# jcorsetti/oryon

Hardware: AMD Instinct MI355X
Metric: image-pairs/sec end-to-end (feat+match+reg) @224², C=256; ADD(-S) parity (higher is better)
Workload: dtype f32

## Files before the change

### include/oryon_hip.h

```cpp
#ifndef ORYON_HIP_H
#define ORYON_HIP_H

#include <stddef.h>
#include <stdint.h>

#ifdef __cplusplus
extern "C" {
#endif

#define ORYON_OK 0
#define ORYON_ERR_INVALID_ARG (-1)
#define ORYON_ERR_HIP (-2)
#define ORYON_ERR_WORKSPACE (-3)
#define ORYON_ERR_NO_DEVICE (-4)
#define ORYON_ERR_STATE (-5)

#define ORYON_PAIR_OK 0
#define ORYON_PAIR_NO_MASK 1
#define ORYON_PAIR_NO_CORR 2

#define ORYON_MATCH_TILE 128

const char *oryon_version(void);
const char *oryon_last_error(void);
// ... 248 lines not shown
    int n_slots;
    int overlap;
    int gather_sets;
    int reg_streams;
    int reg_lag;
    int screen;
    int sample_first;
    int x3_prefetch;
    int stream_roles;
    int screen_cascade;
    int solver;
    int ransac_max_iter;
    float ransac_match_err;
    float ransac_fix_percent;
} oryon_engine_config_t;
size_t oryon_engine_config_bytes(void);
size_t oryon_engine_arena_bytes(const oryon_engine_config_t *cfg, const oryon_pointdsc_t *solver);
int oryon_engine_create(oryon_engine_t **handle, const oryon_engine_config_t *cfg, oryon_pointdsc_t *solver, void *arena,
                        size_t arena_bytes);
void oryon_engine_destroy(oryon_engine_t *handle);
int oryon_engine_warm_streams(void);
int oryon_engine_set_stream_roles(oryon_engine_t *handle, int roles);
int oryon_engine_stream_roles(const oryon_engine_t *handle, int *roles);
int oryon_engine_buffer(const oryon_engine_t *handle, int slot, const char *name, size_t *offset, size_t *bytes);
int oryon_engine_geometry(const oryon_engine_t *handle, int *cap_a, int *cap_q, int *c_pad, int *n_cap);
int oryon_engine_submit(oryon_engine_t *handle, const float *feat_a, const float *feat_q, const int32_t *mask_a, const int32_t *mask_q,
                        const float *depth_a, const float *depth_q, const float *cam_a, const float *cam_q, const int64_t *pair_key,
                        int force_eager, int inputs_resident, void *caller_stream);
int oryon_engine_wait(oryon_engine_t *handle, int slot, void *caller_stream);
int oryon_engine_set_timing(oryon_engine_t *handle, int enable);
int oryon_engine_timing(oryon_engine_t *handle, int64_t step, float *out8);
int oryon_engine_elapsed(oryon_engine_t *handle, int64_t step_a, int event_a, int64_t step_b, int event_b, float *ms);
int oryon_engine_gather_ms(oryon_engine_t *handle, int64_t step, float *ms);
int oryon_engine_host_stats(const oryon_engine_t *handle, int64_t *n_submit, double *submit_ms_total, double *submit_ms_last);
int oryon_engine_x3_steps(const oryon_engine_t *handle, int64_t *n_steps);
int oryon_engine_cascade_stats(oryon_engine_t *handle, int32_t *out);
int oryon_engine_feedback(oryon_engine_t *handle, int64_t *step, int64_t *n_undecided, int64_t *n_anchors);

int oryon_split_f16x3(const float *x, int64_t n, void *hi_f16, void *lo_f16, void *stream);
int oryon_x3_range_flag(int *value_out, int reset, void *stream);
int oryon_linear_f16x3(const float *A, int M, int K, const void *W_hi, const void *W_lo, const float *bias, int N, int act, float *C,
                       void *stream);
int oryon_linear_f16x3_acc(const float *A, int M, int K, const void *W_hi, const void *W_lo, const float *bias, int N, float *C,
                           void *stream);

int oryon_mha_f16x3(const float *qkv, int N, int L, int heads, int head_dim, float *out, void *stream);
// ... 98 lines not shown
```

### oryon_amd/_lib.py

```python
from __future__ import annotations

import ctypes
import os
from ctypes import POINTER, c_char_p, c_float, c_int, c_int64, c_size_t, c_uint64, c_void_p

import torch

_HERE = os.path.dirname(os.path.abspath(__file__))
LIB_PATH = os.path.join(_HERE, "liboryon_hip.so")
_lib = None


class OryonError(RuntimeError):
    pass


class EngineConfig(ctypes.Structure):
    _fields_ = [("B", c_int), ("C", c_int), ("FH", c_int), ("FW", c_int), ("HA", c_int), ("WA", c_int), ("HQ", c_int), ("WQ", c_int),
                ("layout", c_int), ("dist_th", c_float), ("n_corrs", c_int), ("src_sampling", c_int), ("seed", c_uint64),
                ("round_f16", c_int), ("n_slots", c_int), ("overlap", c_int), ("gather_sets", c_int), ("reg_streams", c_int), ("reg_lag", c_int), ("screen", c_int), ("sample_first", c_int), ("x3_prefetch", c_int), ("stream_roles", c_int), ("screen_cascade", c_int),
                ("solver", c_int), ("ransac_max_iter", c_int), ("ransac_match_err", c_float), ("ransac_fix_percent", c_float)]


class DecoderWeights(ctypes.Structure):
# ... 86 lines not shown
                                   _P, _P, _P, _P, _P]),
    "oryon_lift_pairs": (c_int, [_P, _P, c_int, c_int, c_int, c_int, _P, c_int, c_int, _P, c_int, c_int, _P, _P, _P, _P,
                                 _P, _P, _P]),
    "oryon_lift_points": (c_int, [_P, c_int, c_int, _P, _P, _P, c_int, _P, _P]),
    "oryon_kabsch_batched": (c_int, [_P, _P, _P, c_int, c_int, _P, _P]),
    "oryon_split_f16x3": (c_int, [_P, c_int64, _P, _P, _P]),
    "oryon_linear_f16x3": (c_int, [_P, c_int, c_int, _P, _P, _P, c_int, c_int, _P, _P]),
    "oryon_linear_f16x3_acc": (c_int, [_P, c_int, c_int, _P, _P, _P, c_int, _P, _P]),
    "oryon_mha_f16x3": (c_int, [_P, c_int, c_int, c_int, c_int, _P, _P]),
    "oryon_pose_metrics": (c_int, [_P, _P, c_int, _P, _P, c_int, c_int, _P, _P, _P, _P]),
    "oryon_pose_bop_workspace_bytes": (c_size_t, [c_int, c_int]),
    "oryon_pose_bop_errors": (c_int, [_P, _P, _P, c_int, _P, _P, _P, _P, c_int, c_int, _P, c_int, _P, _P, _P]),
    "oryon_render_depth_workspace_bytes": (c_size_t, [c_int, c_int]),
    "oryon_render_depth": (c_int, [_P, _P, c_int, _P, _P, _P, _P, c_int, c_int, _P, c_int, c_int, _P, _P, _P]),
    "oryon_vsd_workspace_bytes": (c_size_t, [c_int, c_int, c_int, c_int]),
    "oryon_vsd_counts": (c_int, [_P, _P, _P, _P, c_int, c_int, c_int, _P, _P, _P, _P, c_int, c_int, _P, _P, ctypes.c_double, _P, c_int,
                                 _P, _P, _P]),
    "oryon_engine_arena_bytes": (c_size_t, [POINTER(EngineConfig), c_void_p]),
    "oryon_engine_create": (c_int, [POINTER(c_void_p), POINTER(EngineConfig), c_void_p, _P, c_size_t]),
    "oryon_engine_destroy": (None, [c_void_p]),
    "oryon_engine_warm_streams": (c_int, []),
    "oryon_engine_set_stream_roles": (c_int, [c_void_p, c_int]),
    "oryon_engine_stream_roles": (c_int, [c_void_p, POINTER(c_int)]),
    "oryon_engine_buffer": (c_int, [c_void_p, c_int, c_char_p, POINTER(c_size_t), POINTER(c_size_t)]),
    "oryon_engine_geometry": (c_int, [c_void_p, POINTER(c_int), POINTER(c_int), POINTER(c_int), POINTER(c_int)]),
    "oryon_engine_submit": (c_int, [c_void_p, _P, _P, _P, _P, _P, _P, _P, _P, _P, c_int, c_int, _P]),
    "oryon_engine_wait": (c_int, [c_void_p, c_int, _P]),
    "oryon_engine_set_timing": (c_int, [c_void_p, c_int]),
    "oryon_engine_timing": (c_int, [c_void_p, c_int64, POINTER(c_float)]),
    "oryon_engine_elapsed": (c_int, [c_void_p, c_int64, c_int, c_int64, c_int, POINTER(c_float)]),
    "oryon_engine_gather_ms": (c_int, [c_void_p, c_int64, POINTER(c_float)]),
    "oryon_engine_config_bytes": (c_size_t, []),
    "oryon_engine_host_stats": (c_int, [c_void_p, POINTER(c_int64), POINTER(ctypes.c_double), POINTER(ctypes.c_double)]),
    "oryon_engine_x3_steps": (c_int, [c_void_p, POINTER(c_int64)]),
    "oryon_engine_cascade_stats": (c_int, [c_void_p, c_void_p]),
    "oryon_engine_feedback": (c_int, [_P, POINTER(c_int64), POINTER(c_int64), POINTER(c_int64)]),
    "oryon_fusion_window_attention_f32": (c_int, [_P, _P, c_int, c_int, c_int, c_int, c_int, c_int, c_int, _P, _P]),
    "oryon_fusion_class_layer_f32": (c_int, [_P, _P, POINTER(FusionClassWeights), c_int, _P, _P]),
    "oryon_conv24_image_bytes": (c_int64, [c_int, c_int, c_int]),
    "oryon_conv24_pack_f16x3": (c_int, [_P, c_int, c_int, c_int, _P, _P]),
    "oryon_conv24_f16x3": (c_int, [_P, c_int, c_int, _P, _P, c_int, c_int, c_int, _P, _P]),
    "oryon_decoder_create": (c_int, [POINTER(DecoderWeights), POINTER(c_void_p), _P]),
    "oryon_decoder_destroy": (None, [c_void_p]),
    "oryon_decoder_workspace_bytes": (c_int64, [c_int, c_int, c_int]),
    "oryon_decoder_workspace_layout": (c_int, [c_int, c_int, c_int, POINTER(c_int64)]),
    "oryon_decoder_forward": (c_int, [c_void_p, _P, _P, _P, c_int, c_int, c_int, _P, c_int64, _P, _P, c_int, c_int, _P]),
# ... 100 lines not shown
```

### oryon_amd/csrc/engine.hip

```cpp
#include <stdlib.h>
#include <chrono>
#include <new>
#include <vector>
#include <string.h>
#include "common.h"
#include "match_common.h"

using namespace oryon;

namespace {
constexpr int MAX_SLOTS = 8;
constexpr int MAX_G_SLOTS = 4;
constexpr int MAX_REG_STREAMS = 4;
constexpr int TIMING_RING = 64;
constexpr int ROW_PAD = 256;
constexpr int POOL_STREAMS = 8;
constexpr int DEFAULT_ROLES = 2345;

inline bool roles_valid(int roles)
{
    if (roles < 0 || roles > 7777) return false;
    for (int d = 0, r = roles; d < 4; ++d, r /= 10)
        if (r % 10 >= POOL_STREAMS) return false;
    return true;
// ... 28 lines not shown

struct Named {
    const char *name;
    size_t off, bytes;
};

struct Layout {
    GatherBuf gbuf[MAX_G_SLOTS];
    SlotBuf slot[MAX_SLOTS];
    std::vector<Named> names[MAX_SLOTS];
    void *match_ws;
    size_t match_ws_bytes, pdsc_ws_bytes, bytes;
    int cap_a, cap_q, c_pad, n_cap, cap_a1;
};
}

struct oryon_engine {
    oryon_engine_config_t cfg;
    oryon_pointdsc_t *solver;
    char *arena;
    Layout L;
    int device;
    hipStream_t sg, sm, sr[MAX_REG_STREAMS];
    int n_reg_streams;
    int roles;
    hipEvent_t ev_inputs[MAX_SLOTS], ev_gathered[MAX_SLOTS], ev_matched[MAX_SLOTS], ev_done[MAX_SLOTS];
    hipEvent_t tev[TIMING_RING][9];
    bool timed[TIMING_RING];
    bool used[MAX_SLOTS];
    bool timing;
    int32_t *fb_host;
    hipEvent_t ev_fb[MAX_SLOTS];
    int64_t fb_step[MAX_SLOTS];
    int64_t fb_seen;
    bool hard_mode;
    int64_t n_x3;
    int64_t n_submit;
    double host_ns_total, host_ns_last;
};

namespace {
int carve_engine(const oryon_engine_config_t &c, const oryon_pointdsc_t *solver, char *base, Layout &L)
{
    const int HW = c.FH * c.FW;
    L.c_pad = c.C <= 256 ? 256 : 512;
    const int keep = c.src_sampling > 0 ? (c.src_sampling < HW ? c.src_sampling : HW) : HW;
    L.cap_a = (int)up((size_t)keep, ROW_PAD);
    L.cap_q = (int)up((size_t)HW, ROW_PAD);
    L.n_cap = (int)up((size_t)c.n_corrs, 128);
// ... 139 lines not shown
        out[i] = pool.all[i];
    }
    return hipSuccess;
}
}

extern "C" int oryon_engine_warm_streams(void)
{
    int dev = 0;
    ORYON_CHECK_HIP(hipGetDevice(&dev));
    hipStream_t tmp[POOL_STREAMS];
    ORYON_CHECK_HIP(acquire_pool(dev, tmp));
    return ORYON_OK;
}

namespace {
int assign_roles(oryon_engine *e, int roles)
{
    hipStream_t pool[POOL_STREAMS];
    ORYON_CHECK_HIP(acquire_pool(e->device, pool));
    const int r_m = roles / 1000 % 10, r_g = roles / 100 % 10, r_r0 = roles / 10 % 10, r_r1 = roles % 10;
    e->sm = e->cfg.overlap >= 1 ? pool[r_m] : nullptr;
    e->sg = e->cfg.overlap >= 2 ? pool[r_g] : nullptr;
    for (int s = 0; s < MAX_REG_STREAMS; ++s) e->sr[s] = nullptr;
    for (int s = 0; s < e->n_reg_streams; ++s)
        if (e->cfg.overlap >= 1) e->sr[s] = pool[(s == 0 ? r_r0 : s == 1 ? r_r1 : 2 + s) & 7];
    e->roles = roles;
    return ORYON_OK;
}
}

extern "C" int oryon_engine_create(oryon_engine_t **handle, const oryon_engine_config_t *cfg, oryon_pointdsc_t *solver, void *arena,
                                   size_t arena_bytes)
{
    ORYON_CHECK_ARG(handle && arena);
    int rc = check_cfg(cfg);
    if (rc) return rc;
    ORYON_CHECK_ARG(solver || cfg->solver == 1);
    oryon_engine *e = new (std::nothrow) oryon_engine();
    ORYON_CHECK_ARG(e != nullptr);
    e->cfg = *cfg;
    e->solver = solver;
    e->arena = static_cast<char *>(arena);
    if ((rc = carve_engine(*cfg, solver, e->arena, e->L))) { delete e; set_error("oryon_engine_create: cannot size the workspaces (solver finalized?)"); return rc; }
    if (arena_bytes < e->L.bytes) {
        set_error("oryon_engine_create: arena too small (%zu < %zu)", arena_bytes, e->L.bytes);
        delete e;
        return ORYON_ERR_WORKSPACE;
    }
    (void)hipGetDevice(&e->device);
    {
        hipPointerAttribute_t attr;
        if (hipPointerGetAttributes(&attr, arena) == hipSuccess && attr.device != e->device) {
            set_error("oryon_engine_create: the arena lives on device %d, the calling thread is on device %d", attr.device, e->device);
            delete e;
            return ORYON_ERR_INVALID_ARG;
        }
        (void)hipGetLastError();
    }
    e->sg = e->sm = nullptr;
    e->timing = false;
    e->n_submit = 0;
    e->fb_host = nullptr;
    e->fb_seen = -1;
    e->hard_mode = false;
    e->n_x3 = 0;
    for (int s = 0; s < MAX_SLOTS; ++s) { e->ev_fb[s] = nullptr; e->fb_step[s] = -1; }
    e->host_ns_total = e->host_ns_last = 0.0;
    hipError_t err = hipSuccess;
    auto ok = [&](hipError_t x) { if (err == hipSuccess) err = x; };
    e->n_reg_streams = cfg->reg_streams;
    for (int s = 0; s < MAX_REG_STREAMS; ++s) e->sr[s] = nullptr;
    if (assign_roles(e, cfg->stream_roles > 0 ? cfg->stream_roles : DEFAULT_ROLES) != ORYON_OK)
        err = hipErrorUnknown;
    for (int s = 0; s < MAX_SLOTS; ++s) {
        e->used[s] = false;
        e->ev_inputs[s] = e->ev_gathered[s] = e->ev_matched[s] = e->ev_done[s] = nullptr;
    }
    for (int r = 0; r < TIMING_RING; ++r) {
        e->timed[r] = false;
        for (int i = 0; i < 9; ++i) e->tev[r][i] = nullptr;
    }
    for (int s = 0; s < cfg->n_slots; ++s) {
        for (hipEvent_t *ev : {&e->ev_inputs[s], &e->ev_gathered[s], &e->ev_matched[s], &e->ev_done[s]})
            ok(hipEventCreateWithFlags(ev, hipEventDisableTiming));
    }
    for (int r = 0; r < TIMING_RING; ++r)
        for (int i = 0; i < 9; ++i) ok(hipEventCreate(&e->tev[r][i]));
    if (cfg->x3_prefetch && e->L.c_pad == 256) {
        ok(hipHostMalloc(reinterpret_cast<void **>(&e->fb_host), (size_t)MAX_SLOTS * 2 * cfg->B * sizeof(int32_t), hipHostMallocDefault));
        for (int s = 0; s < cfg->n_slots; ++s) ok(hipEventCreateWithFlags(&e->ev_fb[s], hipEventDisableTiming));
    }
    for (int s = 0; s < cfg->n_slots; ++s)
        ok(hipMemset(e->L.slot[s].corrs, 0, (size_t)cfg->B * e->L.n_cap * 4 * sizeof(int32_t)));
    ok(hipDeviceSynchronize());
    if (err != hipSuccess) {
        set_error("oryon_engine_create: stream / event creation failed: %s", hipGetErrorString(err));
        oryon_engine_destroy(e);
        return ORYON_ERR_HIP;
    }
    *handle = e;
    return ORYON_OK;
}

extern "C" void oryon_engine_destroy(oryon_engine_t *e)
{
    if (!e) return;
    for (int s = 0; s < MAX_REG_STREAMS; ++s)
        if (e->sr[s]) (void)hipStreamSynchronize(e->sr[s]);
    for (int s = 0; s < MAX_SLOTS; ++s) {
        for (hipEvent_t ev : {e->ev_inputs[s], e->ev_gathered[s], e->ev_matched[s], e->ev_done[s]})
            if (ev) (void)hipEventDestroy(ev);
    }
    for (int r = 0; r < TIMING_RING; ++r)
        for (int i = 0; i < 9; ++i)
            if (e->tev[r][i]) (void)hipEventDestroy(e->tev[r][i]);
    if (e->sm) (void)hipStreamSynchronize(e->sm);
    if (e->sg) (void)hipStreamSynchronize(e->sg);
    for (int s = 0; s < MAX_SLOTS; ++s)
        if (e->ev_fb[s]) (void)hipEventDestroy(e->ev_fb[s]);
    if (e->fb_host) (void)hipHostFree(e->fb_host);
    delete e;
}

extern "C" int oryon_engine_set_timing(oryon_engine_t *e, int enable)
{
    ORYON_CHECK_ARG(e);
    e->timing = enable != 0;
    return ORYON_OK;
}

extern "C" int oryon_engine_set_stream_roles(oryon_engine_t *e, int roles)
{
    ORYON_CHECK_ARG(e && roles_valid(roles));
    if (roles == 0) roles = DEFAULT_ROLES;
    if (e->cfg.overlap == 0 || roles == e->roles) return ORYON_OK;
    for (hipStream_t st : {e->sm, e->sg, e->sr[0], e->sr[1], e->sr[2], e->sr[3]})
        if (st) ORYON_CHECK_HIP(hipStreamSynchronize(st));
    return assign_roles(e, roles);
}

extern "C" int oryon_engine_stream_roles(const oryon_engine_t *e, int *roles)
{
    ORYON_CHECK_ARG(e && roles);
    *roles = e->roles;
    return ORYON_OK;
}

extern "C" int oryon_engine_buffer(const oryon_engine_t *e, int slot, const char *name, size_t *offset, size_t *bytes)
{
    ORYON_CHECK_ARG(e && name && offset && bytes && slot >= 0 && slot < e->cfg.n_slots);
    for (const Named &n : e->L.names[slot])
        if (strcmp(n.name, name) == 0) {
            *offset = n.off;
            *bytes = n.bytes;
            return ORYON_OK;
        }
    set_error("oryon_engine_buffer: no buffer named '%s'", name);
    return ORYON_ERR_INVALID_ARG;
}

extern "C" int oryon_engine_geometry(const oryon_engine_t *e, int *cap_a, int *cap_q, int *c_pad, int *n_cap)
{
    ORYON_CHECK_ARG(e);
    if (cap_a) *cap_a = e->L.cap_a;
    if (cap_q) *cap_q = e->L.cap_q;
    if (c_pad) *c_pad = e->L.c_pad;
    if (n_cap) *n_cap = e->L.n_cap;
    return ORYON_OK;
}

extern "C" int oryon_engine_submit(oryon_engine_t *e, const float *feat_a, const float *feat_q, const int32_t *mask_a, const int32_t *mask_q,
                                   const float *depth_a, const float *depth_q, const float *cam_a, const float *cam_q,
                                   const int64_t *pair_key, int force_eager, int inputs_resident, void *caller_stream)
{
    ORYON_CHECK_ARG(e && feat_a && feat_q && mask_a && mask_q && depth_a && depth_q && cam_a && cam_q);
    const auto t_host0 = std::chrono::steady_clock::now();
    const oryon_engine_config_t &c = e->cfg;
    const int slot = (int)(e->n_submit % c.n_slots);
    SlotBuf &b = e->L.slot[slot];
    GatherBuf &g = e->L.gbuf[e->n_submit % c.gather_sets];
    hipStream_t caller = as_stream(caller_stream);
    hipStream_t sm = c.overlap >= 1 ? e->sm : caller;
    hipStream_t sg = c.overlap >= 2 ? e->sg : sm;
    hipStream_t sr = c.overlap >= 1 ? e->sr[e->n_submit % e->n_reg_streams] : caller;
    const int HW = c.FH * c.FW, B = c.B;
    const bool timing = e->timing;
    hipEvent_t *tev = e->tev[e->n_submit % TIMING_RING];
    e->timed[e->n_submit % TIMING_RING] = timing;
    int rc;
    if (c.overlap >= 1) {
        ORYON_CHECK_HIP(hipEventRecord(e->ev_inputs[slot], caller));
        ORYON_CHECK_HIP(hipStreamWaitEvent(sr, e->ev_inputs[slot], 0));
        if (!inputs_resident || e->n_submit < c.n_slots) {
            ORYON_CHECK_HIP(hipStreamWaitEvent(sg, e->ev_inputs[slot], 0));
            if (sm != sg) ORYON_CHECK_HIP(hipStreamWaitEvent(sm, e->ev_inputs[slot], 0));
        }
        if (e->used[slot]) {
            ORYON_CHECK_HIP(hipStreamWaitEvent(sg, e->ev_done[slot], 0));
            if (sm != sg) ORYON_CHECK_HIP(hipStreamWaitEvent(sm, e->ev_done[slot], 0));
        }
        if (c.reg_lag > 0 && e->n_submit >= c.reg_lag)
            ORYON_CHECK_HIP(hipStreamWaitEvent(sm, e->ev_done[(e->n_submit - c.reg_lag) % c.n_slots], 0));
        if (sg != sm && e->n_submit >= c.gather_sets)
            ORYON_CHECK_HIP(hipStreamWaitEvent(sg, e->ev_matched[(e->n_submit - c.gather_sets) % c.n_slots], 0));
    }
    static const int ablate_env = dev_env_int("ORYON_ENGINE_ABLATE", 0);
    const int ablate = e->n_submit >= (int64_t)(c.n_slots + c.gather_sets) ? ablate_env : 0;
    if (timing) ORYON_CHECK_HIP(hipEventRecord(tev[0], sg));
    const bool mx6 = c.screen == 1 && !force_eager;
    {
        const bool clear = mx6 && !(ablate & 1);
        const bool sf_k0 = e->L.cap_a1 > 0 && !force_eager;
        if ((rc = roi_compact_pair_launch(mask_a, mask_q, B, HW, b.roi_a, b.roi_q, b.n_a, b.n_q, clear ? (sf_k0 ? g.a_eps_1 : g.a_eps) : nullptr,
                                          clear ? g.q_eps : nullptr, sg))) {
            set_error("oryon_engine_submit: roi_compact launch failed");
            return rc;
        }
    }
    if (c.src_sampling > 0 && (rc = oryon_roi_subsample(b.roi_a, b.n_a, B, HW, c.src_sampling, c.seed, pair_key, sg))) return rc;
    const bool sf = e->L.cap_a1 > 0 && !force_eager;
    const int32_t *roi_a_k0 = b.roi_a, *n_a_k0 = b.n_a;
    int cap_a_k0 = e->L.cap_a;
    int8_t *a8_k0 = g.a8;
    float *a_sc_k0 = g.a_sc, *a_eps_k0 = g.a_eps, *a_norm_k0 = g.a_norm, *a_hat_k0 = force_eager ? g.a_hat : nullptr;
    if (sf) {
        ORYON_CHECK_HIP(hipMemcpyAsync(b.roi_a1, b.roi_a, (size_t)B * HW * sizeof(int32_t), hipMemcpyDeviceToDevice, sg));
        ORYON_CHECK_HIP(hipMemcpyAsync(b.n_a1, b.n_a, (size_t)B * sizeof(int32_t), hipMemcpyDeviceToDevice, sg));
        if ((rc = oryon_roi_subsample(b.roi_a1, b.n_a1, B, HW, c.sample_first, c.seed ^ 0x5A17F125ull, pair_key, sg))) return rc;
        roi_a_k0 = b.roi_a1; n_a_k0 = b.n_a1; cap_a_k0 = e->L.cap_a1;
        a8_k0 = g.a8_1; a_sc_k0 = g.a_sc_1; a_eps_k0 = g.a_eps_1; a_norm_k0 = g.a_norm_1;
    }
    bool x3_pre = false;
    if (e->fb_host && mx6) {
        for (int s = 0; s < c.n_slots; ++s) {
            if (e->fb_step[s] > e->fb_seen && hipEventQuery(e->ev_fb[s]) == hipSuccess) {
                const int32_t *h = e->fb_host + (size_t)s * 2 * B;
                long und = 0, all = 0;
                for (int i = 0; i < B; ++i) { und += h[i]; all += h[B + i]; }
                e->hard_mode = all > 0 && 4 * und > all;
                e->fb_seen = e->fb_step[s];
            }
        }
        x3_pre = e->hard_mode && !sf && g.q_hilo != nullptr;
    }
    if (x3_pre) a_hat_k0 = g.a_hat;
    if (timing) ORYON_CHECK_HIP(hipEventRecord(tev[8], sg));
    if (ablate & 1) {
    } else if (mx6) {
        if (x3_pre) {
            if ((rc = oryon_gather_mx6_x3(feat_q, B, c.C, HW, c.layout, b.roi_q, HW, b.n_q, e->L.cap_q, e->L.c_pad, reinterpret_cast<uint8_t *>(g.q8),
                                          g.q_eps, g.q_norm, g.q_hilo, g.q_lo_max, c.round_f16, sg))) return rc;
            e->n_x3 += 1;
        } else
        if ((rc = gather_mx6_prezeroed(feat_q, B, c.C, HW, c.layout, b.roi_q, HW, b.n_q, e->L.cap_q, e->L.c_pad, reinterpret_cast<uint8_t *>(g.q8),
                                       g.q_eps, g.q_norm, nullptr, c.round_f16, sg))) return rc;
        if ((rc = gather_mx6_prezeroed(feat_a, B, c.C, HW, c.layout, roi_a_k0, HW, n_a_k0, cap_a_k0, e->L.c_pad, reinterpret_cast<uint8_t *>(a8_k0),
                                       a_eps_k0, a_norm_k0, a_hat_k0, c.round_f16, sg))) return rc;
    } else {
    if ((rc = oryon_gather_q8(feat_q, B, c.C, HW, c.layout, b.roi_q, HW, b.n_q, e->L.cap_q, e->L.c_pad, g.q8, g.q_sc, g.q_eps, g.q_norm,
                              nullptr, c.round_f16, sg))) return rc;
    if ((rc = oryon_gather_q8(feat_a, B, c.C, HW, c.layout, roi_a_k0, HW, n_a_k0, cap_a_k0, e->L.c_pad, a8_k0, a_sc_k0, a_eps_k0, a_norm_k0,
                              a_hat_k0, c.round_f16, sg))) return rc;
    }
    if (timing) ORYON_CHECK_HIP(hipEventRecord(tev[1], sg));
    if (sg != sm) {
        ORYON_CHECK_HIP(hipEventRecord(e->ev_gathered[slot], sg));
        ORYON_CHECK_HIP(hipStreamWaitEvent(sm, e->ev_gathered[slot], 0));
    }
    struct Disarm {
        bool armed = false;
        ~Disarm() { if (armed) (void)oryon_profile_events(nullptr, nullptr); }
    } disarm;
    if (timing) {
        ORYON_CHECK_HIP(hipEventRecord(tev[2], sm));
        (void)oryon_profile_events(tev[4], tev[5]);
        disarm.armed = true;
    }
    auto match_call = [&](const float *a_norm_, const int8_t *a8_, const float *a_sc_, const float *a_eps_, const int32_t *roi_a_, int cap_a_,
                          const int32_t *n_a_, int32_t *corrs_, int32_t *n_valid_, int32_t *n_sel_, int32_t *status_, int32_t *n_und_) -> int {
        MatchCorrsArgs m;
        m.a_i8 = a8_;
        m.a_scale = mx6 ? a_eps_ : a_sc_;
        m.roi_a = roi_a_;
        m.roi_stride_a = HW;
        m.feat_q = feat_q;
        m.q_norm = g.q_norm;
        m.roi_q = b.roi_q;
        m.roi_stride_q = HW;
        m.q_i8 = g.q8;
        m.q_scale = mx6 ? nullptr : g.q_sc;
        m.q_eps_max = g.q_eps;
        m.C_true = c.C;
        m.HW = HW;
        m.layout = c.layout;
        m.B = B;
        m.C = e->L.c_pad;
        m.cap_a = cap_a_;
        m.cap_q = e->L.cap_q;
        m.round_f16 = c.round_f16;
        m.n_a = n_a_;
        m.n_q = b.n_q;
        m.threshold = c.dist_th;
// ... 6 lines not shown
        m.argmin = b.argmin;
        m.valid = b.valid;
        m.corrs = corrs_;
        m.n_valid = n_valid_;
        m.n_sel = n_sel_;
        m.status = status_;
        m.n_undecided = n_und_;
        m.workspace = e->L.match_ws;
        m.workspace_bytes = e->L.match_ws_bytes;
        m.stream = sm;
        m.fmt = mx6 ? 1 : 0;
        m.cascade = (c.screen_cascade && !sf) ? 1 : 0;
        if (mx6 && x3_pre) {
            m.a_hat = g.a_hat;
            m.q_hi_lo = g.q_hilo;
            m.q_lo_sq_max = g.q_lo_max;
        } else if (force_eager) {
            m.a_hat = g.a_hat;
            m.force_eager = force_eager;
        } else {
            m.feat_a = feat_a;
            m.a_norm = a_norm_;
        }
        return match_corrs_lazy_impl(m);
    };
    if (ablate & 2) {
    } else if (sf) {
        if ((rc = match_call(g.a_norm_1, g.a8_1, g.a_sc_1, g.a_eps_1, b.roi_a1, e->L.cap_a1, b.n_a1, b.corrs, b.n_valid, b.n_sel, b.status, b.n_und)))
            return rc;
        if ((rc = oryon_sample_first_gate(b.n_valid, b.n_a1, b.n_a, B, c.n_corrs, b.n_a2, sm))) return rc;
        if (mx6) {
            if ((rc = oryon_gather_mx6(feat_a, B, c.C, HW, c.layout, b.roi_a, HW, b.n_a2, e->L.cap_a, e->L.c_pad, reinterpret_cast<uint8_t *>(g.a8),
                                       g.a_eps, g.a_norm, nullptr, c.round_f16, sm))) return rc;
        } else if ((rc = oryon_gather_q8(feat_a, B, c.C, HW, c.layout, b.roi_a, HW, b.n_a2, e->L.cap_a, e->L.c_pad, g.a8, g.a_sc, g.a_eps, g.a_norm,
                                         nullptr, c.round_f16, sm))) return rc;
        if ((rc = match_call(g.a_norm, g.a8, g.a_sc, g.a_eps, b.roi_a, e->L.cap_a, b.n_a2, b.corrs2, b.n_valid2, b.n_sel2, b.status2, nullptr)))
            return rc;
        if ((rc = oryon_sample_first_merge(b.n_a2, b.corrs2, b.n_valid2, b.n_sel2, b.status2, B, e->L.n_cap, b.corrs, b.n_valid, b.n_sel, b.status,
                                           sm))) return rc;
    } else if ((rc = match_call(g.a_norm, g.a8, g.a_sc, g.a_eps, b.roi_a, e->L.cap_a, b.n_a, b.corrs, b.n_valid, b.n_sel, b.status, b.n_und)))
        return rc;
    if (e->fb_host && mx6 && !(ablate & 2)) {
        int32_t *h = e->fb_host + (size_t)slot * 2 * B;
        ORYON_CHECK_HIP(hipMemcpyAsync(h, b.n_und, (size_t)B * sizeof(int32_t), hipMemcpyDeviceToHost, sm));
        ORYON_CHECK_HIP(hipMemcpyAsync(h + B, b.n_a, (size_t)B * sizeof(int32_t), hipMemcpyDeviceToHost, sm));
        ORYON_CHECK_HIP(hipEventRecord(e->ev_fb[slot], sm));
        e->fb_step[slot] = e->n_submit;
    }
    if (!(ablate & 2) && (rc = oryon_lift_pairs(b.corrs, b.n_sel, B, e->L.n_cap, c.FH, c.FW, depth_a, c.HA, c.WA, depth_q, c.HQ, c.WQ, cam_a, cam_q,
                                                b.status, b.pcd_a, b.pcd_q, b.n_lift, sm))) return rc;
    if (timing) ORYON_CHECK_HIP(hipEventRecord(tev[3], sm));
    if (c.overlap >= 1) {
        ORYON_CHECK_HIP(hipEventRecord(e->ev_matched[slot], sm));
        ORYON_CHECK_HIP(hipStreamWaitEvent(sr, e->ev_matched[slot], 0));
    }
    if (timing) ORYON_CHECK_HIP(hipEventRecord(tev[6], sr));
    if (c.solver == 1) {
        if (!(ablate & 4) && (rc = oryon_ransac_register(b.pcd_a, b.pcd_q, b.n_lift, B, e->L.n_cap, c.ransac_max_iter, (double)c.ransac_match_err,
                                                         (double)c.ransac_fix_percent, nullptr, c.seed, pair_key, b.status, b.pdsc_ws,
                                                         e->L.pdsc_ws_bytes, b.pose, nullptr, nullptr, nullptr, b.status_out, sr))) return rc;
    } else if (!(ablate & 4) && (rc = oryon_pointdsc_register(e->solver, b.pcd_a, b.pcd_q, b.n_lift, B, e->L.n_cap, b.status, b.pdsc_ws, e->L.pdsc_ws_bytes,
                                                       b.pose, nullptr, b.status_out, sr))) return rc;
    hipLaunchKernelGGL(engine_counts_kernel, dim3((B + 255) / 256), dim3(256), 0, sr, b.n_valid, b.n_lift, B, b.n_valid_out, b.n_lift_out);
    ORYON_CHECK_LAUNCH();
    if (timing) ORYON_CHECK_HIP(hipEventRecord(tev[7], sr));
    if (c.overlap >= 1) ORYON_CHECK_HIP(hipEventRecord(e->ev_done[slot], sr));
    e->used[slot] = true;
    e->n_submit += 1;
// ... 95 lines not shown
```

### oryon_amd/csrc/match_common.h

```cpp
#pragma once
#include <hip/hip_fp16.h>
#include "common.h"

namespace oryon {

typedef float f32x16 __attribute__((ext_vector_type(16)));

__device__ __forceinline__ void lex_min(float &d, int &i, float od, int oi)
{
    const bool take = (od < d) || (od == d && oi < i);
    d = take ? od : d;
    i = take ? oi : i;
}

int match_f32_flagged(const float *a_hat, const float *q_hat, int B, int C, int cap_a, int cap_q, const int32_t *n_a,
                      const int32_t *n_q, float threshold, float *min_dist, int32_t *argmin, uint8_t *valid,
                      const int32_t *panel_flag, const uint8_t *row_flag, void *stream);

int match_f32_split(int B, int T);

size_t match_x3_scratch_bytes(int B, int cap_s, int S, int cap_q);
size_t match_x3_zero_bytes(int B, int cap_s, int S);
int match_x3_resolve(const float *a_c, const int32_t *n_c, int cap_s, const float *feat_q, int C_true, int HW, int layout,
                     const int32_t *roi_q, int roi_stride_q, const float *q_norm, const int32_t *n_q, int B, int cap_q, float threshold,
// ... 151 lines not shown
struct MatchCorrsArgs : Screen8Args {
    const float *feat_a = nullptr;
    const float *a_norm = nullptr;
    const int32_t *roi_a = nullptr;
    int roi_stride_a = 0;
    const void *q_hi_lo = nullptr;
    const float *q_lo_sq_max = nullptr;
    const int32_t *n_a = nullptr;
    int W = 0;
    int max_corrs = 0;
    int corr_rows = 0;
    uint64_t seed = 0;
    const int64_t *pair_key = nullptr;
    int32_t *corrs = nullptr;
    int32_t *n_valid = nullptr;
    int32_t *n_sel = nullptr;
    int32_t *status = nullptr;
    int32_t *n_undecided = nullptr;
    void *workspace = nullptr;
    size_t workspace_bytes = 0;
    int fmt = 0;
    int force_eager = 0;
    int cascade = 1;
};
int match_corrs_lazy_impl(const MatchCorrsArgs &m);
int32_t *match_dc_stats(void *workspace, int B, int C, int cap_a, int cap_q, int corr_rows);

}
```

### oryon_amd/csrc/match_corrs.hip

```cpp
#include <hip/hip_fp16.h>
#include "common.h"
#include "match_common.h"
#include "match_exact.h"

namespace oryon {
constexpr uint8_t LZ_INVALID = 0, LZ_VALID = 1, LZ_UNCERTAIN = 2, LZ_AMB_VALID = 3, LZ_RESOLVED = 4, LZ_AMB_UNCERTAIN = 5;
constexpr uint8_t DC_COMPLETE = 0, DC_SETTLED = 1, DC_OPEN = 2;

struct DcOpenRows {
    const uint8_t *cls = nullptr;
    int S = 0;
    const float *m1 = nullptr;
    const int32_t *i1 = nullptr;
    const float *m2 = nullptr;
    float *r_m1 = nullptr;
    int32_t *r_i1 = nullptr;
    float *r_m2 = nullptr;
};

__device__ __forceinline__ bool decide_lite_row(
    int cap_a, int p, int a, int S, const float *ws_m1, const int32_t *ws_i1,
    const float *ws_m2, const DcOpenRows &open, const float *__restrict__ a_scale8, const float *__restrict__ eps_q8, float cut0, float sqrt_c,
    float c_true, int force_eager, int fmt, int x3, float *__restrict__ m_final, int32_t *__restrict__ sid_final, float *__restrict__ margin_out,
    uint8_t *__restrict__ state, uint8_t *__restrict__ valid, float *__restrict__ min_dist, int32_t *__restrict__ argmin,
// ... 60 lines not shown
    if (force_eager) return;
    const unsigned long long amb_lanes = __ballot(amb);
    if ((threadIdx.x & 63) == 0) s_amb[threadIdx.x >> 6] = __popcll(amb_lanes);
    __syncthreads();
    if (threadIdx.x == 0) n_amb_part[(size_t)p * gridDim.x + blockIdx.x] = s_amb[0] + s_amb[1] + s_amb[2] + s_amb[3];
}

__device__ __forceinline__ int amb_total(const int32_t *__restrict__ n_amb_part, int n_parts, int p)
{
    int tot = 0;
    for (int i = 0; i < n_parts; ++i) tot += n_amb_part[(size_t)p * n_parts + i];
    return tot;
}

__global__ void match_mask_counts_kernel(int B, const int32_t *__restrict__ n_a, const int32_t *__restrict__ pair_eager,
                                         int32_t *__restrict__ n_a_eager, int32_t *__restrict__ n_a_lazy)
{
    const int p = blockIdx.x * blockDim.x + threadIdx.x;
    if (p >= B) return;
    n_a_eager[p] = pair_eager[p] ? n_a[p] : 0;
    n_a_lazy[p] = pair_eager[p] ? 0 : n_a[p];
}

__global__ void match_cascade_counts_kernel(int B, const int32_t *__restrict__ n_amb_part, int n_parts, const int32_t *__restrict__ n_after,
                                            const int32_t *__restrict__ n_before, int32_t *__restrict__ out)
{
    const int p = blockIdx.x * blockDim.x + threadIdx.x;
    if (p >= B) return;
    const long long tot = amb_total(n_amb_part, n_parts, p), nb = n_before[p], na = n_after[p];
    out[p] = nb > 0 ? (int32_t)(tot * na / nb) : (int32_t)tot;
}

__global__ void match_sum_counts_kernel(int B, const int32_t *__restrict__ a, const int32_t *__restrict__ n_amb_part, int n_parts,
                                        int32_t *__restrict__ out)
{
    const int p = blockIdx.x * blockDim.x + threadIdx.x;
    if (p < B) out[p] = a[p] + amb_total(n_amb_part, n_parts, p);
}

__global__ __launch_bounds__(256) void match_compact_f32_kernel(const float *__restrict__ a_hat, int Cp, int cap_a, int cap_c,
                                                                 const int32_t *__restrict__ count, const int32_t *__restrict__ idx,
                                                                 int idx_stride, float *__restrict__ a_c)
{
    const int p = blockIdx.y, lane = threadIdx.x & 63;
    const int n = count[p] < cap_c ? count[p] : cap_c;
    const int n_fill = (n + 127) / 128 * 128;
    for (int g = 0; g < 16; ++g) {
        const int sl = (blockIdx.x * 16 + g) * 4 + (threadIdx.x >> 6);
        if (sl >= n_fill || sl >= cap_c) break;
        uint4 *d = reinterpret_cast<uint4 *>(a_c + ((size_t)p * cap_c + sl) * Cp);
        if (sl >= n) {
            for (int i = lane; i < Cp / 4; i += 64) d[i] = make_uint4(0, 0, 0, 0);
            continue;
        }
        const uint4 *src = reinterpret_cast<const uint4 *>(a_hat + ((size_t)p * cap_a + idx[(size_t)p * idx_stride + sl]) * Cp);
        for (int i = lane; i < Cp / 4; i += 64) d[i] = src[i];
    }
}

__global__ __launch_bounds__(256) void match_scatter_exact_kernel(int cap_a, int cap_c, const int32_t *__restrict__ count,
// ... 623 lines not shown
                           cap_s, w.x3_a_ovf);
        if ((rc = check_launch(IMPL))) return rc;
        rc = oryon_match_f32(w.x3_a_ovf, w.q_hat, B, C, cap_s, cap_q, n_ovf, m.n_q, m.threshold, w.x3_md_o, w.x3_am_o, w.x3_va_o, w.exact_ws,
                             w.exact_ws_bytes, st);
        if (rc) return rc;
        match_x3_scatter_ovf(B, cap_s, n_ovf, ovf_idx, w.x3_md_o, w.x3_am_o, w.x3_va_o, w.md_c, w.am_c, w.va_c, st);
    } else {
        rc = oryon_match_f32(w.a_hat_c, w.q_hat, B, C, cap_s, cap_q, w.n_ambv, m.n_q, m.threshold, w.md_c, w.am_c, w.va_c, w.exact_ws,
                             w.exact_ws_bytes, st);
        if (rc) return rc;
    }
    hipLaunchKernelGGL(match_scatter_exact_kernel, dim3((cap_s + 255) / 256, B), dim3(256), 0, st, cap_a, cap_s, w.n_ambv, w.ambv_idx,
                       corr_rows, w.md_c, w.am_c, w.va_c, m.min_dist, m.argmin, m.valid, w.state);
    if ((rc = check_launch(IMPL))) return rc;
    auto resolve_selected = m.fmt == 1 ? (nhwc ? match_resolve_selected_kernel<true, 1> : match_resolve_selected_kernel<false, 1>)
                                       : (nhwc ? match_resolve_selected_kernel<true, 0> : match_resolve_selected_kernel<false, 0>);
    hipLaunchKernelGGL(resolve_selected, dim3((m.max_corrs + 3) / 4, B), dim3(256), lds_res, st, m.a_hat, araw, m.a_i8, m.q_i8, m.q_scale,
                       m.a_scale, m.feat_q, m.C_true, m.HW, m.roi_q, m.roi_stride_q, m.q_norm, C, cap_a, cap_q, m.n_q, m.W, w.m_final,
                       w.sid_final, w.margin, w.state, w.pair_eager, m.n_sel, w.sel_rows, corr_rows, m.min_dist, m.argmin, m.corrs,
                       m.round_f16);
    if ((rc = check_launch(IMPL))) return rc;
    if (m.n_undecided && cascade) {
        hipLaunchKernelGGL(match_cascade_counts_kernel, dim3((B + 255) / 256), dim3(256), 0, st, B, w.n_amb_part, cap_a / 256, w.n_ambv, w.n_ambv0,
                           m.n_undecided);
        if ((rc = check_launch(IMPL))) return rc;
    } else if (m.n_undecided) {
        hipLaunchKernelGGL(match_sum_counts_kernel, dim3((B + 255) / 256), dim3(256), 0, st, B, w.n_amb, w.n_amb_part, cap_a / 256,
                           m.n_undecided);
        if ((rc = check_launch(IMPL))) return rc;
    }
    return ORYON_OK;
}
}

int oryon::match_corrs_lazy_impl(const MatchCorrsArgs &m)
{
    ORYON_CHECK_ARG((m.a_hat || (m.feat_a && m.a_norm && !m.force_eager)) && m.a_i8 && m.a_scale && m.feat_q && m.roi_a && m.roi_q && m.q_norm && m.q_i8 && m.q_eps_max && m.n_a && m.n_q);
    ORYON_CHECK_ARG((m.fmt == 0 || m.fmt == 1) && (m.fmt == 1 || m.q_scale) && !(m.fmt == 1 && m.force_eager));
    ORYON_CHECK_ARG(!m.q_hi_lo || (m.q_lo_sq_max && m.C == 256));
    ORYON_CHECK_ARG(m.min_dist && m.argmin && m.valid && m.corrs && m.n_valid && m.n_sel && m.status);
    ORYON_CHECK_ARG(m.B >= 0 && (m.C == 256 || m.C == 512) && m.C_true > 0 && m.C_true <= m.C && m.HW > 0 && m.W > 0 && m.max_corrs > 0 && m.corr_rows >= m.max_corrs);
    ORYON_CHECK_ARG(m.layout == ORYON_LAYOUT_NCHW || m.layout == ORYON_LAYOUT_NHWC);
    ORYON_CHECK_ARG(m.cap_a > 0 && m.cap_a % MT16 == 0 && m.cap_q > 0 && m.cap_q % 256 == 0 && m.threshold > 0.0f && m.threshold <= 0.5f);
    if (m.B == 0) return ORYON_OK;
    const int B = m.B, C = m.C, cap_a = m.cap_a, cap_q = m.cap_q;
    const int T = cap_a / MT16;
    const int S = pick_split16(B, T);
    LazyWs w;
    const size_t need = carve_lazy(m.workspace, w, B, C, cap_a, cap_q, S, m.corr_rows);
    ORYON_CHECK_WORKSPACE("oryon_match_corrs_i8: ", m.workspace, m.workspace_bytes, need);
    hipStream_t st = as_stream(m.stream);
// ... 245 lines not shown
```

Before: 23980.

## Move ROI prep to dedicated stream and write feedback counts from kernels

Adds a dedicated prep stream that runs ROI compaction, subsampling and the sample-first copies, then signals the gather stream through a per-slot event. This lets the next submit's ROI preparation overlap with gather work already queued. It also removes two device-to-host memcpys of the feedback counts by having the count kernels write directly into the pinned host buffer. The cost is an extra stream and event per slot, plus zero-copy writes to host memory from the device.

```diff
diff --git a/include/oryon_hip.h b/include/oryon_hip.h
--- a/include/oryon_hip.h
+++ b/include/oryon_hip.h
@@ -294,6 +294,7 @@
 int oryon_engine_warm_streams(void);
 int oryon_engine_set_stream_roles(oryon_engine_t *handle, int roles);
 int oryon_engine_stream_roles(const oryon_engine_t *handle, int *roles);
+int oryon_engine_prep_stream(const oryon_engine_t *handle, int *pool_position);
 int oryon_engine_buffer(const oryon_engine_t *handle, int slot, const char *name, size_t *offset, size_t *bytes);
 int oryon_engine_geometry(const oryon_engine_t *handle, int *cap_a, int *cap_q, int *c_pad, int *n_cap);
 int oryon_engine_submit(oryon_engine_t *handle, const float *feat_a, const float *feat_q, const int32_t *mask_a, const int32_t *mask_q,
diff --git a/oryon_amd/_lib.py b/oryon_amd/_lib.py
--- a/oryon_amd/_lib.py
+++ b/oryon_amd/_lib.py
@@ -132,6 +132,7 @@
     "oryon_engine_warm_streams": (c_int, []),
     "oryon_engine_set_stream_roles": (c_int, [c_void_p, c_int]),
     "oryon_engine_stream_roles": (c_int, [c_void_p, POINTER(c_int)]),
+    "oryon_engine_prep_stream": (c_int, [c_void_p, POINTER(c_int)]),
     "oryon_engine_buffer": (c_int, [c_void_p, c_int, c_char_p, POINTER(c_size_t), POINTER(c_size_t)]),
     "oryon_engine_geometry": (c_int, [c_void_p, POINTER(c_int), POINTER(c_int), POINTER(c_int), POINTER(c_int)]),
     "oryon_engine_submit": (c_int, [c_void_p, _P, _P, _P, _P, _P, _P, _P, _P, _P, c_int, c_int, _P]),
diff --git a/oryon_amd/csrc/engine.hip b/oryon_amd/csrc/engine.hip
--- a/oryon_amd/csrc/engine.hip
+++ b/oryon_amd/csrc/engine.hip
@@ -74,9 +74,12 @@
     Layout L;
     int device;
     hipStream_t sg, sm, sr[MAX_REG_STREAMS];
+    hipStream_t sp;
     int n_reg_streams;
     int roles;
+    int prep_pos;
     hipEvent_t ev_inputs[MAX_SLOTS], ev_gathered[MAX_SLOTS], ev_matched[MAX_SLOTS], ev_done[MAX_SLOTS];
+    hipEvent_t ev_rois[MAX_SLOTS];
     hipEvent_t tev[TIMING_RING][9];
     bool timed[TIMING_RING];
     bool used[MAX_SLOTS];
@@ -262,6 +265,10 @@
     const int r_m = roles / 1000 % 10, r_g = roles / 100 % 10, r_r0 = roles / 10 % 10, r_r1 = roles % 10;
     e->sm = e->cfg.overlap >= 1 ? pool[r_m] : nullptr;
     e->sg = e->cfg.overlap >= 2 ? pool[r_g] : nullptr;
+    int pos = 0;
+    while (pos == r_m || pos == r_g || pos == r_r0 || pos == r_r1) ++pos;
+    e->prep_pos = pos;
+    e->sp = e->cfg.overlap >= 2 ? pool[pos] : nullptr;
     for (int s = 0; s < MAX_REG_STREAMS; ++s) e->sr[s] = nullptr;
     for (int s = 0; s < e->n_reg_streams; ++s)
         if (e->cfg.overlap >= 1) e->sr[s] = pool[(s == 0 ? r_r0 : s == 1 ? r_r1 : 2 + s) & 7];
@@ -298,7 +305,8 @@
         }
         (void)hipGetLastError();
     }
-    e->sg = e->sm = nullptr;
+    e->sg = e->sm = e->sp = nullptr;
+    e->prep_pos = -1;
     e->timing = false;
     e->n_submit = 0;
     e->fb_host = nullptr;
@@ -315,14 +323,14 @@
         err = hipErrorUnknown;
     for (int s = 0; s < MAX_SLOTS; ++s) {
         e->used[s] = false;
-        e->ev_inputs[s] = e->ev_gathered[s] = e->ev_matched[s] = e->ev_done[s] = nullptr;
+        e->ev_inputs[s] = e->ev_gathered[s] = e->ev_matched[s] = e->ev_done[s] = e->ev_rois[s] = nullptr;
     }
     for (int r = 0; r < TIMING_RING; ++r) {
         e->timed[r] = false;
         for (int i = 0; i < 9; ++i) e->tev[r][i] = nullptr;
     }
     for (int s = 0; s < cfg->n_slots; ++s) {
-        for (hipEvent_t *ev : {&e->ev_inputs[s], &e->ev_gathered[s], &e->ev_matched[s], &e->ev_done[s]})
+        for (hipEvent_t *ev : {&e->ev_inputs[s], &e->ev_gathered[s], &e->ev_matched[s], &e->ev_done[s], &e->ev_rois[s]})
             ok(hipEventCreateWithFlags(ev, hipEventDisableTiming));
     }
     for (int r = 0; r < TIMING_RING; ++r)
@@ -349,7 +357,7 @@
     for (int s = 0; s < MAX_REG_STREAMS; ++s)
         if (e->sr[s]) (void)hipStreamSynchronize(e->sr[s]);
     for (int s = 0; s < MAX_SLOTS; ++s) {
-        for (hipEvent_t ev : {e->ev_inputs[s], e->ev_gathered[s], e->ev_matched[s], e->ev_done[s]})
+        for (hipEvent_t ev : {e->ev_inputs[s], e->ev_gathered[s], e->ev_matched[s], e->ev_done[s], e->ev_rois[s]})
             if (ev) (void)hipEventDestroy(ev);
     }
     for (int r = 0; r < TIMING_RING; ++r)
@@ -357,6 +365,7 @@
             if (e->tev[r][i]) (void)hipEventDestroy(e->tev[r][i]);
     if (e->sm) (void)hipStreamSynchronize(e->sm);
     if (e->sg) (void)hipStreamSynchronize(e->sg);
+    if (e->sp) (void)hipStreamSynchronize(e->sp);
     for (int s = 0; s < MAX_SLOTS; ++s)
         if (e->ev_fb[s]) (void)hipEventDestroy(e->ev_fb[s]);
     if (e->fb_host) (void)hipHostFree(e->fb_host);
@@ -375,9 +384,16 @@
     ORYON_CHECK_ARG(e && roles_valid(roles));
     if (roles == 0) roles = DEFAULT_ROLES;
     if (e->cfg.overlap == 0 || roles == e->roles) return ORYON_OK;
-    for (hipStream_t st : {e->sm, e->sg, e->sr[0], e->sr[1], e->sr[2], e->sr[3]})
+    for (hipStream_t st : {e->sm, e->sg, e->sp, e->sr[0], e->sr[1], e->sr[2], e->sr[3]})
         if (st) ORYON_CHECK_HIP(hipStreamSynchronize(st));
     return assign_roles(e, roles);
+}
+
+extern "C" int oryon_engine_prep_stream(const oryon_engine_t *e, int *pool_position)
+{
+    ORYON_CHECK_ARG(e && pool_position);
+    *pool_position = e->sp ? e->prep_pos : -1;
+    return ORYON_OK;
 }
 
 extern "C" int oryon_engine_stream_roles(const oryon_engine_t *e, int *roles)
@@ -424,6 +440,7 @@
     hipStream_t sm = c.overlap >= 1 ? e->sm : caller;
     hipStream_t sg = c.overlap >= 2 ? e->sg : sm;
     hipStream_t sr = c.overlap >= 1 ? e->sr[e->n_submit % e->n_reg_streams] : caller;
+    hipStream_t sp = c.overlap >= 2 ? e->sp : sg;
     const int HW = c.FH * c.FW, B = c.B;
     const bool timing = e->timing;
     hipEvent_t *tev = e->tev[e->n_submit % TIMING_RING];
@@ -433,41 +450,41 @@
         ORYON_CHECK_HIP(hipEventRecord(e->ev_inputs[slot], caller));
         ORYON_CHECK_HIP(hipStreamWaitEvent(sr, e->ev_inputs[slot], 0));
         if (!inputs_resident || e->n_submit < c.n_slots) {
-            ORYON_CHECK_HIP(hipStreamWaitEvent(sg, e->ev_inputs[slot], 0));
+            ORYON_CHECK_HIP(hipStreamWaitEvent(sp, e->ev_inputs[slot], 0));
             if (sm != sg) ORYON_CHECK_HIP(hipStreamWaitEvent(sm, e->ev_inputs[slot], 0));
         }
         if (e->used[slot]) {
-            ORYON_CHECK_HIP(hipStreamWaitEvent(sg, e->ev_done[slot], 0));
+            ORYON_CHECK_HIP(hipStreamWaitEvent(sp, e->ev_done[slot], 0));
             if (sm != sg) ORYON_CHECK_HIP(hipStreamWaitEvent(sm, e->ev_done[slot], 0));
         }
         if (c.reg_lag > 0 && e->n_submit >= c.reg_lag)
             ORYON_CHECK_HIP(hipStreamWaitEvent(sm, e->ev_done[(e->n_submit - c.reg_lag) % c.n_slots], 0));
         if (sg != sm && e->n_submit >= c.gather_sets)
-            ORYON_CHECK_HIP(hipStreamWaitEvent(sg, e->ev_matched[(e->n_submit - c.gather_sets) % c.n_slots], 0));
+            ORYON_CHECK_HIP(hipStreamWaitEvent(sp, e->ev_matched[(e->n_submit - c.gather_sets) % c.n_slots], 0));
     }
     static const int ablate_env = dev_env_int("ORYON_ENGINE_ABLATE", 0);
     const int ablate = e->n_submit >= (int64_t)(c.n_slots + c.gather_sets) ? ablate_env : 0;
-    if (timing) ORYON_CHECK_HIP(hipEventRecord(tev[0], sg));
+    if (timing && sp == sg) ORYON_CHECK_HIP(hipEventRecord(tev[0], sg));
     const bool mx6 = c.screen == 1 && !force_eager;
     {
         const bool clear = mx6 && !(ablate & 1);
         const bool sf_k0 = e->L.cap_a1 > 0 && !force_eager;
         if ((rc = roi_compact_pair_launch(mask_a, mask_q, B, HW, b.roi_a, b.roi_q, b.n_a, b.n_q, clear ? (sf_k0 ? g.a_eps_1 : g.a_eps) : nullptr,
-                                          clear ? g.q_eps : nullptr, sg))) {
+                                          clear ? g.q_eps : nullptr, sp))) {
             set_error("oryon_engine_submit: roi_compact launch failed");
             return rc;
         }
     }
-    if (c.src_sampling > 0 && (rc = oryon_roi_subsample(b.roi_a, b.n_a, B, HW, c.src_sampling, c.seed, pair_key, sg))) return rc;
+    if (c.src_sampling > 0 && (rc = oryon_roi_subsample(b.roi_a, b.n_a, B, HW, c.src_sampling, c.seed, pair_key, sp))) return rc;
     const bool sf = e->L.cap_a1 > 0 && !force_eager;
     const int32_t *roi_a_k0 = b.roi_a, *n_a_k0 = b.n_a;
     int cap_a_k0 = e->L.cap_a;
     int8_t *a8_k0 = g.a8;
     float *a_sc_k0 = g.a_sc, *a_eps_k0 = g.a_eps, *a_norm_k0 = g.a_norm, *a_hat_k0 = force_eager ? g.a_hat : nullptr;
     if (sf) {
-        ORYON_CHECK_HIP(hipMemcpyAsync(b.roi_a1, b.roi_a, (size_t)B * HW * sizeof(int32_t), hipMemcpyDeviceToDevice, sg));
-        ORYON_CHECK_HIP(hipMemcpyAsync(b.n_a1, b.n_a, (size_t)B * sizeof(int32_t), hipMemcpyDeviceToDevice, sg));
-        if ((rc = oryon_roi_subsample(b.roi_a1, b.n_a1, B, HW, c.sample_first, c.seed ^ 0x5A17F125ull, pair_key, sg))) return rc;
+        ORYON_CHECK_HIP(hipMemcpyAsync(b.roi_a1, b.roi_a, (size_t)B * HW * sizeof(int32_t), hipMemcpyDeviceToDevice, sp));
+        ORYON_CHECK_HIP(hipMemcpyAsync(b.n_a1, b.n_a, (size_t)B * sizeof(int32_t), hipMemcpyDeviceToDevice, sp));
+        if ((rc = oryon_roi_subsample(b.roi_a1, b.n_a1, B, HW, c.sample_first, c.seed ^ 0x5A17F125ull, pair_key, sp))) return rc;
         roi_a_k0 = b.roi_a1; n_a_k0 = b.n_a1; cap_a_k0 = e->L.cap_a1;
         a8_k0 = g.a8_1; a_sc_k0 = g.a_sc_1; a_eps_k0 = g.a_eps_1; a_norm_k0 = g.a_norm_1;
     }
@@ -485,6 +502,11 @@
         x3_pre = e->hard_mode && !sf && g.q_hilo != nullptr;
     }
     if (x3_pre) a_hat_k0 = g.a_hat;
+    if (sp != sg) {
+        ORYON_CHECK_HIP(hipEventRecord(e->ev_rois[slot], sp));
+        ORYON_CHECK_HIP(hipStreamWaitEvent(sg, e->ev_rois[slot], 0));
+        if (timing) ORYON_CHECK_HIP(hipEventRecord(tev[0], sg));
+    }
     if (timing) ORYON_CHECK_HIP(hipEventRecord(tev[8], sg));
     if (ablate & 1) {
     } else if (mx6) {
@@ -508,17 +530,8 @@
         ORYON_CHECK_HIP(hipEventRecord(e->ev_gathered[slot], sg));
         ORYON_CHECK_HIP(hipStreamWaitEvent(sm, e->ev_gathered[slot], 0));
     }
-    struct Disarm {
-        bool armed = false;
-        ~Disarm() { if (armed) (void)oryon_profile_events(nullptr, nullptr); }
-    } disarm;
-    if (timing) {
-        ORYON_CHECK_HIP(hipEventRecord(tev[2], sm));
-        (void)oryon_profile_events(tev[4], tev[5]);
-        disarm.armed = true;
-    }
-    auto match_call = [&](const float *a_norm_, const int8_t *a8_, const float *a_sc_, const float *a_eps_, const int32_t *roi_a_, int cap_a_,
-                          const int32_t *n_a_, int32_t *corrs_, int32_t *n_valid_, int32_t *n_sel_, int32_t *status_, int32_t *n_und_) -> int {
+    auto match_args = [&](const float *a_norm_, const int8_t *a8_, const float *a_sc_, const float *a_eps_, const int32_t *roi_a_, int cap_a_,
+                          const int32_t *n_a_, int32_t *corrs_, int32_t *n_valid_, int32_t *n_sel_, int32_t *status_, int32_t *n_und_) -> MatchCorrsArgs {
         MatchCorrsArgs m;
         m.a_i8 = a8_;
         m.a_scale = mx6 ? a_eps_ : a_sc_;
@@ -571,28 +584,39 @@
             m.feat_a = feat_a;
             m.a_norm = a_norm_;
         }
-        return match_corrs_lazy_impl(m);
+        if (n_und_ && e->fb_host && mx6) {
+            m.fb_counts = e->fb_host + (size_t)slot * 2 * B;
+            m.fb_n_a = b.n_a;
+        }
+        return m;
     };
+    MatchCorrsArgs m1 = sf ? match_args(g.a_norm_1, g.a8_1, g.a_sc_1, g.a_eps_1, b.roi_a1, e->L.cap_a1, b.n_a1, b.corrs, b.n_valid, b.n_sel, b.status, b.n_und)
+                           : match_args(g.a_norm, g.a8, g.a_sc, g.a_eps, b.roi_a, e->L.cap_a, b.n_a, b.corrs, b.n_valid, b.n_sel, b.status, b.n_und);
+    struct Disarm {
+        bool armed = false;
+        ~Disarm() { if (armed) (void)oryon_profile_events(nullptr, nullptr); }
+    } disarm;
+    if (timing) {
+        ORYON_CHECK_HIP(hipEventRecord(tev[2], sm));
+        (void)oryon_profile_events(tev[4], tev[5]);
+        disarm.armed = true;
+    }
     if (ablate & 2) {
     } else if (sf) {
-        if ((rc = match_call(g.a_norm_1, g.a8_1, g.a_sc_1, g.a_eps_1, b.roi_a1, e->L.cap_a1, b.n_a1, b.corrs, b.n_valid, b.n_sel, b.status, b.n_und)))
-            return rc;
+        if ((rc = match_corrs_lazy_impl(m1))) return rc;
         if ((rc = oryon_sample_first_gate(b.n_valid, b.n_a1, b.n_a, B, c.n_corrs, b.n_a2, sm))) return rc;
         if (mx6) {
             if ((rc = oryon_gather_mx6(feat_a, B, c.C, HW, c.layout, b.roi_a, HW, b.n_a2, e->L.cap_a, e->L.c_pad, reinterpret_cast<uint8_t *>(g.a8),
                                        g.a_eps, g.a_norm, nullptr, c.round_f16, sm))) return rc;
         } else if ((rc = oryon_gather_q8(feat_a, B, c.C, HW, c.layout, b.roi_a, HW, b.n_a2, e->L.cap_a, e->L.c_pad, g.a8, g.a_sc, g.a_eps, g.a_norm,
                                          nullptr, c.round_f16, sm))) return rc;
-        if ((rc = match_call(g.a_norm, g.a8, g.a_sc, g.a_eps, b.roi_a, e->L.cap_a, b.n_a2, b.corrs2, b.n_valid2, b.n_sel2, b.status2, nullptr)))
-            return rc;
+        if ((rc = match_corrs_lazy_impl(match_args(g.a_norm, g.a8, g.a_sc, g.a_eps, b.roi_a, e->L.cap_a, b.n_a2, b.corrs2, b.n_valid2, b.n_sel2, b.status2,
+                                                   nullptr)))) return rc;
         if ((rc = oryon_sample_first_merge(b.n_a2, b.corrs2, b.n_valid2, b.n_sel2, b.status2, B, e->L.n_cap, b.corrs, b.n_valid, b.n_sel, b.status,
                                            sm))) return rc;
-    } else if ((rc = match_call(g.a_norm, g.a8, g.a_sc, g.a_eps, b.roi_a, e->L.cap_a, b.n_a, b.corrs, b.n_valid, b.n_sel, b.status, b.n_und)))
+    } else if ((rc = match_corrs_lazy_impl(m1)))
         return rc;
     if (e->fb_host && mx6 && !(ablate & 2)) {
-        int32_t *h = e->fb_host + (size_t)slot * 2 * B;
-        ORYON_CHECK_HIP(hipMemcpyAsync(h, b.n_und, (size_t)B * sizeof(int32_t), hipMemcpyDeviceToHost, sm));
-        ORYON_CHECK_HIP(hipMemcpyAsync(h + B, b.n_a, (size_t)B * sizeof(int32_t), hipMemcpyDeviceToHost, sm));
         ORYON_CHECK_HIP(hipEventRecord(e->ev_fb[slot], sm));
         e->fb_step[slot] = e->n_submit;
     }
diff --git a/oryon_amd/csrc/match_common.h b/oryon_amd/csrc/match_common.h
--- a/oryon_amd/csrc/match_common.h
+++ b/oryon_amd/csrc/match_common.h
@@ -197,6 +197,8 @@
     int fmt = 0;
     int force_eager = 0;
     int cascade = 1;
+    int32_t *fb_counts = nullptr;
+    const int32_t *fb_n_a = nullptr;
 };
 int match_corrs_lazy_impl(const MatchCorrsArgs &m);
 int32_t *match_dc_stats(void *workspace, int B, int C, int cap_a, int cap_q, int corr_rows);
diff --git a/oryon_amd/csrc/match_corrs.hip b/oryon_amd/csrc/match_corrs.hip
--- a/oryon_amd/csrc/match_corrs.hip
+++ b/oryon_amd/csrc/match_corrs.hip
@@ -106,20 +106,33 @@
     n_a_lazy[p] = pair_eager[p] ? 0 : n_a[p];
 }
 
+__device__ __forceinline__ void store_feedback(int32_t *fb_counts, const int32_t *fb_n_a, int B, int p, int32_t und)
+{
+    if (!fb_counts) return;
+    fb_counts[p] = und;
+    fb_counts[B + p] = fb_n_a[p];
+}
+
 __global__ void match_cascade_counts_kernel(int B, const int32_t *__restrict__ n_amb_part, int n_parts, const int32_t *__restrict__ n_after,
-                                            const int32_t *__restrict__ n_before, int32_t *__restrict__ out)
+                                            const int32_t *__restrict__ n_before, int32_t *__restrict__ out, int32_t *__restrict__ fb_counts,
+                                            const int32_t *__restrict__ fb_n_a)
 {
     const int p = blockIdx.x * blockDim.x + threadIdx.x;
     if (p >= B) return;
     const long long tot = amb_total(n_amb_part, n_parts, p), nb = n_before[p], na = n_after[p];
-    out[p] = nb > 0 ? (int32_t)(tot * na / nb) : (int32_t)tot;
+    const int32_t und = nb > 0 ? (int32_t)(tot * na / nb) : (int32_t)tot;
+    out[p] = und;
+    store_feedback(fb_counts, fb_n_a, B, p, und);
 }
 
 __global__ void match_sum_counts_kernel(int B, const int32_t *__restrict__ a, const int32_t *__restrict__ n_amb_part, int n_parts,
-                                        int32_t *__restrict__ out)
+                                        int32_t *__restrict__ out, int32_t *__restrict__ fb_counts, const int32_t *__restrict__ fb_n_a)
 {
     const int p = blockIdx.x * blockDim.x + threadIdx.x;
-    if (p < B) out[p] = a[p] + amb_total(n_amb_part, n_parts, p);
+    if (p >= B) return;
+    const int32_t und = a[p] + amb_total(n_amb_part, n_parts, p);
+    out[p] = und;
+    store_feedback(fb_counts, fb_n_a, B, p, und);
 }
 
 __global__ __launch_bounds__(256) void match_compact_f32_kernel(const float *__restrict__ a_hat, int Cp, int cap_a, int cap_c,
@@ -789,11 +802,11 @@
     if ((rc = check_launch(IMPL))) return rc;
     if (m.n_undecided && cascade) {
         hipLaunchKernelGGL(match_cascade_counts_kernel, dim3((B + 255) / 256), dim3(256), 0, st, B, w.n_amb_part, cap_a / 256, w.n_ambv, w.n_ambv0,
-                           m.n_undecided);
+                           m.n_undecided, m.fb_counts, m.fb_n_a);
         if ((rc = check_launch(IMPL))) return rc;
     } else if (m.n_undecided) {
         hipLaunchKernelGGL(match_sum_counts_kernel, dim3((B + 255) / 256), dim3(256), 0, st, B, w.n_amb, w.n_amb_part, cap_a / 256,
-                           m.n_undecided);
+                           m.n_undecided, m.fb_counts, m.fb_n_a);
         if ((rc = check_launch(IMPL))) return rc;
     }
     return ORYON_OK;
```

After: 23490. -2.1%, worse.
